# chanchanchan97/ICAFusion

Hardware: AMD Instinct MI355X
Metric: RGB/IR image-pairs/sec (two-stream forward + NMS) (higher is better)
Workload: dtype bf16

## Files before the change

### icafusion_amd/csrc/cstream.hip

```cpp
#include "conv_common.h"

namespace icaf {

constexpr int CS_C = 64, CS_TH = 8, CS_TW = 16, CS_HH = CS_TH + 2, CS_HWD = CS_TW + 2, CS_PITCH = 24;
constexpr int CS_NIDX = CS_HH * CS_PITCH;
constexpr int CS_PATCH = CS_NIDX * 128;
constexpr int CS_WBYTES = 9 * CS_C * 128;
constexpr int CS_W2BYTES = CS_C * 128;
constexpr int CS_SO = CS_C * 2 + 16;
constexpr int CS_STG = 128 * CS_SO;
constexpr int CS_LDS = CS_WBYTES + CS_W2BYTES + 2 * CS_PATCH + CS_STG;
static_assert(CS_LDS <= 160 * 1024, "LDS capacity");

struct CsGeom { int tiles_x, tiles_y, ntile; };

template <int DT, bool CHAIN>
__global__ __launch_bounds__(512) __attribute__((amdgpu_waves_per_eu(2, 2))) void cstream_kernel(const ConvP p, const CsGeom gm) {
    using E = Elem<DT>;
    static_assert(DT != ICAF_F32, "16-bit types");
    constexpr int RB = 128, NSTEP = 4, VEC = E::VEC;
    extern __shared__ __attribute__((aligned(1024))) unsigned char lds[];
    unsigned char* wbuf = lds;
    unsigned char* w2buf = lds + CS_WBYTES;
    unsigned char* patch0 = w2buf + CS_W2BYTES;
    unsigned char* stg = patch0 + 2 * CS_PATCH;

    const int tid = threadIdx.x, lane = tid & 63, l31 = lane & 31, hi = lane >> 5;
    const int wave = __builtin_amdgcn_readfirstlane(tid >> 6);
    const int g = blockIdx.z;
    const int wm = wave & 3, wn = wave >> 2;
    const int sy = wm >> 1, sx = wm & 1;

    const __amdgpu_buffer_rsrc_t xr = __builtin_amdgcn_make_buffer_rsrc(
        (void*)((const typename E::type*)p.x + g * p.x_gs), 0, p.x_bytes, 0x00020000);
    const __amdgpu_buffer_rsrc_t wr = __builtin_amdgcn_make_buffer_rsrc(
        (void*)((const typename E::type*)p.w + g * p.w_gs), 0, p.w_bytes, 0x00020000);
    constexpr unsigned OOB = 0x80000000u;

    {
        const int rsub = lane >> 3;
        for (int t = wave; t < 72; t += 8) {
            const int c = t >> 3, j = t & 7;
            const int sl = (lane & 7) ^ (((j & 1) << 2) | (rsub >> 1));
            const unsigned voff = ((unsigned)(j * 8 + rsub) * (unsigned)p.Kp + (unsigned)(c * 64 + sl * VEC)) * E::BYTES;
            __builtin_amdgcn_raw_ptr_buffer_load_lds(wr, (lds_ptr_t)(wbuf + (c * 64 + j * 8) * RB), 16, voff, 0, 0, 0);
        }
        if constexpr (CHAIN) {
            const __amdgpu_buffer_rsrc_t w2r = __builtin_amdgcn_make_buffer_rsrc(
                (void*)((const typename E::type*)p.w2 + g * p.w2_gs), 0, p.w2_bytes, 0x00020000);
            const int j = wave;
            const int sl = (lane & 7) ^ (((j & 1) << 2) | (rsub >> 1));
            const unsigned voff = ((unsigned)(j * 8 + rsub) * (unsigned)p.Kp2 + (unsigned)(sl * VEC)) * E::BYTES;
            __builtin_amdgcn_raw_ptr_buffer_load_lds(w2r, (lds_ptr_t)(w2buf + (j * 8) * RB), 16, voff, 0, 0, 0);
        }
    }

    const int xcd = blockIdx.x & 7, lb = blockIdx.x >> 3, wgx = gridDim.x >> 3;
    const int per_xcd = (gm.ntile + 7) >> 3, t_lo = xcd * per_xcd, t_hi = min(t_lo + per_xcd, gm.ntile);
    const int per_img = gm.tiles_x * gm.tiles_y;
    auto decode = [&](int t, int& b, int& y0, int& x0) {
        b = t / per_img;
        const int r = t - b * per_img, ty = r / gm.tiles_x;
        y0 = ty * CS_TH;
        x0 = (r - ty * gm.tiles_x) * CS_TW;
    };
    auto issue_patch = [&](int t, int buf) {
        int b, y0, x0;
        decode(t, b, y0, x0);
        const unsigned img_off = (unsigned)b * (unsigned)(p.H * p.W) * (unsigned)p.ldx * (unsigned)E::BYTES;
        unsigned char* dst = patch0 + buf * CS_PATCH;
        for (int j = wave; j < CS_PATCH / 1024; j += 8) {
            const int L = (j << 6) + lane, idx = L >> 3;
            const int cs = (L & 7) ^ ((idx >> 1) & 7);
            const int hy = idx / CS_PITCH, hx = idx - hy * CS_PITCH;
            const int gy = y0 - 1 + hy, gx = x0 - 1 + hx;
            const bool ok = hx < CS_HWD && (unsigned)gy < (unsigned)p.H && (unsigned)gx < (unsigned)p.W;
            const unsigned voff = ok ? img_off + (unsigned)((gy * p.W + gx) * p.ldx) * E::BYTES + (unsigned)(cs << 4) : OOB;
            __builtin_amdgcn_raw_ptr_buffer_load_lds(xr, (lds_ptr_t)(dst + (j << 10)), 16, voff, 0, 0, 0);
        }
    };

    f32x4 bq[4], bq2[4];
    {
        const float* __restrict__ bias = p.bias ? p.bias + g * p.bias_gs : nullptr;
        const float* __restrict__ bias2 = (CHAIN && p.bias2) ? p.bias2 + g * p.bias2_gs : nullptr;
#pragma unroll
        for (int qd = 0; qd < 4; ++qd) {
            const int n = wn * 32 + 8 * qd + 4 * hi;
            const f32x4 t1 = *(const f32x4*)((bias && n < p.Cout) ? bias + n : (const float*)p.w);
            bq[qd] = (bias && n < p.Cout) ? t1 : f32x4{0.f, 0.f, 0.f, 0.f};
            const f32x4 t2 = *(const f32x4*)((bias2 && n < p.Cout2) ? bias2 + n : (const float*)p.w);
            bq2[qd] = (bias2 && n < p.Cout2) ? t2 : f32x4{0.f, 0.f, 0.f, 0.f};
        }
#pragma unroll
        for (int qd = 0; qd < 4; ++qd) asm volatile("" : "+v"(bq[qd]), "+v"(bq2[qd]));
    }
    const int fkey = (l31 >> 1) & 7;
    int foff[NSTEP];
#pragma unroll
    for (int s = 0; s < NSTEP; ++s) foff[s] = (wn * 32 + l31) * RB + (((2 * s + hi) ^ fkey) << 4);
    const int lpy = sy * 4 + (l31 >> 3), lpx = sx * 8 + (l31 & 7);
    const int lbase = lpy * CS_PITCH + lpx;
    const int srow = wm * 32 + l31;

    int t = t_lo + lb;
    if (t >= t_hi) { wait_vmcnt<0>(); return; }
    issue_patch(t, 0);

    typename E::type* __restrict__ yg = (typename E::type*)p.y + g * p.y_gs;
    const typename E::type* __restrict__ rg = p.res ? (const typename E::type*)p.res + g * p.res_gs : nullptr;
    typename E::type* __restrict__ y2g = CHAIN ? (typename E::type*)p.y2 + g * p.y2_gs : nullptr;
    const float alpha_acc = p.alpha_acc[g], alpha_res = p.alpha_res[g];

    auto row_to_m = [&](int r, int b, int y0, int x0) {
        const int st = r >> 5, q = r & 31;
        const int gy = y0 + (st >> 1) * 4 + (q >> 3), gx = x0 + (st & 1) * 8 + (q & 7);
        return (gy < p.Ho && gx < p.Wo) ? (b * p.Ho + gy) * p.Wo + gx : -1;
    };
    u32x4 rres[2] = {u32x4{0u, 0u, 0u, 0u}, u32x4{0u, 0u, 0u, 0u}};
    auto flush = [&](typename E::type* dst, int ldd, int cout, int b, int y0, int x0, bool rr) {
#pragma unroll
        for (int it = 0; it < 2; ++it) {
            const int idx = tid + it * 512, row = idx >> 3, cv = idx & 7;
            const int m = row_to_m(row, b, y0, x0), n = cv * VEC;
            if (m >= 0 && n < cout) {
                u32x4 sv = *(const u32x4*)(stg + row * CS_SO + cv * 16);
                if (rr) {
                    float v[VEC], r[VEC];
                    unpack16<DT>(sv, v);
                    unpack16<DT>(rres[it], r);
#pragma unroll
                    for (int j = 0; j < VEC; ++j) v[j] = __builtin_fmaf(alpha_res, r[j], v[j]);
                    sv = pack16<DT>(v);
                }
                *(u32x4*)(dst + (long long)m * ldd + n) = sv;
            }
        }
    };
    auto load_res = [&](int b, int y0, int x0) {
#pragma unroll
        for (int it = 0; it < 2; ++it) {
            const int idx = tid + it * 512, row = idx >> 3, cv = idx & 7;
            const int m = row_to_m(row, b, y0, x0);
            rres[it] = *(const u32x4*)(rg + (long long)(m < 0 ? 0 : m) * p.ldr + cv * VEC);
        }
    };
    auto stage = [&](const f32x16& acc, const f32x4 (&bv)[4], float scale) {
#pragma unroll
        for (int qd = 0; qd < 4; ++qd) {
            const int nl = wn * 32 + 8 * qd + 4 * hi;
            float v[4];
#pragma unroll
            for (int j = 0; j < 4; ++j) v[j] = acc[4 * qd + j] + bv[qd][j] + 0.0f;
            silu4_f(v, v);
#pragma unroll
            for (int j = 0; j < 4; ++j) v[j] *= scale;
            u32x2 pk;
            if constexpr (DT == ICAF_BF16) { pk[0] = pack2_bf16(v[0], v[1]); pk[1] = pack2_bf16(v[2], v[3]); }
            else { pk[0] = pack2_f16(v[0], v[1]); pk[1] = pack2_f16(v[2], v[3]); }
            *(u32x2*)(stg + srow * CS_SO + nl * E::BYTES) = pk;
        }
    };

    int cur = 0, pb = -1, py0 = 0, px0 = 0;
    while (true) {
        int b, y0, x0;
        decode(t, b, y0, x0);
        const int tn = t + wgx;
        wait_vmcnt<0>();
        asm volatile("s_waitcnt lgkmcnt(0)" ::: "memory");
        __builtin_amdgcn_s_barrier();
        if (pb >= 0) {
            if constexpr (CHAIN) flush(y2g, p.ldy2, p.Cout2, pb, py0, px0, false);
            else flush(yg, p.ldy, p.Cout, pb, py0, px0, rg != nullptr);
        }
        if (rg) load_res(b, y0, x0);
        if (tn < t_hi) issue_patch(tn, cur ^ 1);
        const unsigned char* patch = patch0 + cur * CS_PATCH;
        f32x16 acc;
#pragma unroll
        for (int r = 0; r < 16; ++r) acc[r] = 0.0f;
#pragma unroll
        for (int c = 0; c < 9; ++c) {
            const int ky = c / 3, kx = c - 3 * ky;
            const int idx = lbase + ky * CS_PITCH + kx;
            const unsigned char* pe = patch + (idx << 7);
            const int key = (idx >> 1) & 7;
#pragma unroll
            for (int s = 0; s < NSTEP; ++s) {
                const u32x4 fp = *(const u32x4*)(pe + (((2 * s + hi) ^ key) << 4));
                const u32x4 fw = *(const u32x4*)(wbuf + c * (CS_C * RB) + foff[s]);
                mma_step<DT>(acc, fw, fp);
            }
        }
        lds_barrier();
        stage(acc, bq, alpha_acc);
        pb = b; py0 = y0; px0 = x0;
        if constexpr (CHAIN) {
            lds_barrier();
            if (rg) { wait_vmcnt<0>(); }
#pragma unroll
            for (int it = 0; it < 2; ++it) {
                const int idx = tid + it * 512, row = idx >> 3, cv = idx & 7;
                const int m = row_to_m(row, b, y0, x0), n = cv * VEC;
                if (m >= 0 && n < p.Cout) {
                    u32x4 sv = *(const u32x4*)(stg + row * CS_SO + cv * 16);
                    if (rg) {
                        float v[VEC], r[VEC];
                        unpack16<DT>(sv, v);
                        unpack16<DT>(rres[it], r);
#pragma unroll
                        for (int j = 0; j < VEC; ++j) v[j] = __builtin_fmaf(alpha_res, r[j], v[j]);
                        sv = pack16<DT>(v);
                        *(u32x4*)(stg + row * CS_SO + cv * 16) = sv;
                    }
                    if (p.keep1) *(u32x4*)(yg + (long long)m * p.ldy + n) = sv;
                }
            }
            lds_barrier();
            f32x16 acc2;
#pragma unroll
            for (int r = 0; r < 16; ++r) acc2[r] = 0.0f;
#pragma unroll
            for (int s = 0; s < NSTEP; ++s) {
                const u32x4 fp2 = *(const u32x4*)(stg + srow * CS_SO + ((2 * s + hi) << 4));
                const u32x4 fw2 = *(const u32x4*)(w2buf + foff[s]);
                mma_step<DT>(acc2, fw2, fp2);
            }
            lds_barrier();
            stage(acc2, bq2, 1.0f);
        }
        if (tn >= t_hi) break;
        t = tn;
        cur ^= 1;
    }
    wait_vmcnt<0>();
    lds_barrier();
    if constexpr (CHAIN) flush(y2g, p.ldy2, p.Cout2, pb, py0, px0, false);
    else flush(yg, p.ldy, p.Cout, pb, py0, px0, rg != nullptr);
}

const char* cstream_tag(int) { return "8x16n64"; }

int cstream_check(const icaf_conv_args* a, const ConvP& p, int) {
    if (a->dtype == ICAF_F32 || a->out_dtype != a->dtype) return fail(ICAF_ERR_UNSUPPORTED, "cstream: 16-bit types, out dtype == dtype");
    if (a->kh != 3 || a->kw != 3 || a->sh != 1 || a->sw != 1 || a->ph != 1 || a->pw != 1) return fail(ICAF_ERR_UNSUPPORTED, "cstream: 3x3 / stride 1 / pad 1 layers");
    if (a->Cin != CS_C || a->Cout > CS_C || a->Cout % 8 || a->Kp != 9 * CS_C) return fail(ICAF_ERR_UNSUPPORTED, "cstream: built for 64 -> (<= 64) channels (Cin = %d, Cout = %d, Kp = %d)", a->Cin, a->Cout, a->Kp);
    if (a->act != ICAF_ACT_SILU || a->pre) return fail(ICAF_ERR_UNSUPPORTED, "cstream: SiLU layers without a pre-activation term");
    if (p.x_bytes == 0) return fail(ICAF_ERR_UNSUPPORTED, "cstream: operand exceeds the 2 GiB buffer-descriptor range");
    if (!p.vec_y || (a->res && !p.vec_r)) return fail(ICAF_ERR_UNSUPPORTED, "cstream: y / res must take 16-byte vectors");
    if (a->w2) {
        if (a->Cout2 > CS_C || a->Cout2 % 8 || a->Kp2 != CS_C || !p.vec_y2 || a->Cout != CS_C) return fail(ICAF_ERR_UNSUPPORTED, "cstream: chained 1x1 of 64 -> (<= 64) channels with Kp2 = 64");
        if (a->res && !a->chain_keep) return fail(ICAF_ERR_UNSUPPORTED, "cstream: a residual needs chain_keep");
        if (a->chain_keep && (a->alpha_acc[0] != 1.0f || a->alpha_acc[1] != 1.0f)) return fail(ICAF_ERR_UNSUPPORTED, "cstream: chain_keep with alpha_acc != 1");
    }
    return ICAF_OK;
}

template <int DT, bool CHAIN>
static int launch_cstream_cfg(const ConvP& p, int groups, hipStream_t s) {
    CsGeom gm;
    gm.tiles_x = (p.Wo + CS_TW - 1) / CS_TW;
    gm.tiles_y = (p.Ho + CS_TH - 1) / CS_TH;
    gm.ntile = p.B * gm.tiles_x * gm.tiles_y;
    int dev = 0, cus = 256;
    ICAF_HIP(hipGetDevice(&dev));
    ICAF_HIP(hipDeviceGetAttribute(&cus, hipDeviceAttributeMultiprocessorCount, dev));
    int grid = (cus / groups) & ~7;
    if (grid < 8) grid = 8;
    ICAF_LDS_OPTIN((cstream_kernel<DT, CHAIN>), CS_LDS);
    cstream_kernel<DT, CHAIN><<<dim3((unsigned)grid, 1, (unsigned)groups), dim3(512), CS_LDS, s>>>(p, gm);
    ICAF_LAUNCH_CHECK();
    return ICAF_OK;
}

int launch_cstream(const icaf_conv_args* a, const ConvP& p, int, hipStream_t s) {
    if (a->dtype == ICAF_BF16) return a->w2 ? launch_cstream_cfg<ICAF_BF16, true>(p, a->groups, s) : launch_cstream_cfg<ICAF_BF16, false>(p, a->groups, s);
    return a->w2 ? launch_cstream_cfg<ICAF_F16, true>(p, a->groups, s) : launch_cstream_cfg<ICAF_F16, false>(p, a->groups, s);
}

}
```

Before: 16840.

## Incremental tile walk, precomputed patch/flush offsets, software-pipelined LDS fragment loads

Replaces the per-tile divide-based tile decode with an incremental walker, and precomputes the per-lane patch DMA and flush/residual offsets so each tile only adds a base offset. Unrolls the tile loop over two compile-time buffer indices so LDS addresses fold into immediates. Double-buffers the weight and patch fragment reads in the 9-tap MMA loop, prefetching the next tap's operands behind the current MFMA with sched barriers. It also adds an optional clock-stamp probe build and a phase-timing script. The aim is to cut scalar/VALU address overhead and hide LDS read latency, at the cost of more live VGPRs under a 2-waves-per-EU limit.

```diff
diff --git a/icafusion_amd/csrc/cs_walk.h b/icafusion_amd/csrc/cs_walk.h
--- /dev/null
+++ b/icafusion_amd/csrc/cs_walk.h
@@ -0,0 +1,94 @@
+#pragma once
+
+#if defined(__HIPCC__) || defined(__CUDACC__)
+#define ICAF_CS_HD __host__ __device__ __forceinline__
+#else
+#define ICAF_CS_HD inline
+#endif
+
+namespace icaf {
+
+constexpr int CSW_TH = 8, CSW_TW = 16, CSW_HH = CSW_TH + 2, CSW_HWD = CSW_TW + 2, CSW_PITCH = 24;
+constexpr int CSW_NDMA = CSW_HH * CSW_PITCH * 128 / 1024;
+constexpr int CSW_NEVER = 0x40000000;
+constexpr unsigned CSW_OOB = 0x80000000u;
+
+struct CsWalk {
+    int t, t_hi, stride;
+    int img, ty, tx;
+    int s_img, s_ty, s_tx;
+    int tiles_x, tiles_y;
+};
+
+ICAF_CS_HD bool cs_walk_start(CsWalk& w, int ntile, int tiles_x, int tiles_y, int xcd, int lb, int wgx) {
+    const int per_xcd = (ntile + 7) >> 3, t_lo = xcd * per_xcd;
+    w.t_hi = t_lo + per_xcd < ntile ? t_lo + per_xcd : ntile;
+    w.t = t_lo + lb;
+    w.stride = wgx;
+    w.tiles_x = tiles_x;
+    w.tiles_y = tiles_y;
+    if (w.t >= w.t_hi) return false;
+    const int per_img = tiles_x * tiles_y;
+    w.img = w.t / per_img;
+    int r = w.t - w.img * per_img;
+    w.ty = r / tiles_x;
+    w.tx = r - w.ty * tiles_x;
+    w.s_img = wgx / per_img;
+    r = wgx - w.s_img * per_img;
+    w.s_ty = r / tiles_x;
+    w.s_tx = r - w.s_ty * tiles_x;
+    return true;
+}
+
+ICAF_CS_HD bool cs_walk_has_next(const CsWalk& w) { return w.t + w.stride < w.t_hi; }
+
+ICAF_CS_HD void cs_walk_next(CsWalk& w) {
+    w.t += w.stride;
+    w.tx += w.s_tx;
+    if (w.tx >= w.tiles_x) { w.tx -= w.tiles_x; ++w.ty; }
+    w.ty += w.s_ty;
+    if (w.ty >= w.tiles_y) { w.ty -= w.tiles_y; ++w.img; }
+    w.img += w.s_img;
+}
+
+struct CsPatchLane {
+    int hy1, hx1;
+    unsigned rel;
+};
+
+ICAF_CS_HD CsPatchLane cs_patch_lane(int j, int lane, int W, int pix_bytes) {
+    const int L = (j << 6) + lane, idx = L >> 3;
+    const int cs = (L & 7) ^ ((idx >> 1) & 7);
+    const int hy = idx / CSW_PITCH, hx = idx - hy * CSW_PITCH;
+    CsPatchLane pl;
+    pl.hy1 = hy - 1;
+    pl.hx1 = hx < CSW_HWD ? hx - 1 : CSW_NEVER;
+    pl.rel = hx < CSW_HWD ? (unsigned)((pl.hy1 * W + pl.hx1) * pix_bytes) + (unsigned)(cs << 4) : 0u;
+    return pl;
+}
+
+ICAF_CS_HD unsigned cs_tile_off(int img, int y0, int x0, int H, int W, int pix_bytes) {
+    return ((unsigned)img * (unsigned)(H * W) + (unsigned)(y0 * W + x0)) * (unsigned)pix_bytes;
+}
+
+ICAF_CS_HD unsigned cs_patch_voff(const CsPatchLane& pl, unsigned tile_off, int y0, int x0, int H, int W) {
+    const bool ok = (unsigned)(y0 + pl.hy1) < (unsigned)H && (unsigned)(x0 + pl.hx1) < (unsigned)W;
+    return ok ? tile_off + pl.rel : CSW_OOB;
+}
+
+struct CsFlushLane { int dy, dx, cv; };
+
+ICAF_CS_HD CsFlushLane cs_flush_lane(int tid, int it) {
+    const int idx = tid + it * 512, row = idx >> 3, st = row >> 5, q = row & 31;
+    return CsFlushLane{(st >> 1) * 4 + (q >> 3), (st & 1) * 8 + (q & 7), idx & 7};
+}
+
+ICAF_CS_HD int cs_frag_direct(int lbase, int ky, int kx, int s, int hi) {
+    const int idx = lbase + ky * CSW_PITCH + kx;
+    return (idx << 7) + (((2 * s + hi) ^ ((idx >> 1) & 7)) << 4);
+}
+ICAF_CS_HD int cs_frag_base(int lbase, int kx, int s, int hi) { return cs_frag_direct(lbase, 0, kx, s, hi); }
+constexpr int cs_frag_sel(int ky, int s) { return (ky & 1) ? (s ^ 2) : s; }
+constexpr int cs_frag_imm(int ky) { return ky * CSW_PITCH * 128; }
+
+}
diff --git a/icafusion_amd/csrc/cstream.hip b/icafusion_amd/csrc/cstream.hip
--- a/icafusion_amd/csrc/cstream.hip
+++ b/icafusion_amd/csrc/cstream.hip
@@ -1,8 +1,13 @@
 #include "conv_common.h"
+#include "cs_walk.h"
+#include <type_traits>
+#ifdef ICAF_CS_CLK
+#include <cstdlib>
+#endif
 
 namespace icaf {
 
-constexpr int CS_C = 64, CS_TH = 8, CS_TW = 16, CS_HH = CS_TH + 2, CS_HWD = CS_TW + 2, CS_PITCH = 24;
+constexpr int CS_C = 64, CS_TH = CSW_TH, CS_TW = CSW_TW, CS_HH = CSW_HH, CS_HWD = CSW_HWD, CS_PITCH = CSW_PITCH;
 constexpr int CS_NIDX = CS_HH * CS_PITCH;
 constexpr int CS_PATCH = CS_NIDX * 128;
 constexpr int CS_WBYTES = 9 * CS_C * 128;
@@ -11,8 +16,21 @@
 constexpr int CS_STG = 128 * CS_SO;
 constexpr int CS_LDS = CS_WBYTES + CS_W2BYTES + 2 * CS_PATCH + CS_STG;
 static_assert(CS_LDS <= 160 * 1024, "LDS capacity");
-
-struct CsGeom { int tiles_x, tiles_y, ntile; };
+static_assert(CS_PATCH == CSW_NDMA * 1024, "patch DMA instructions");
+
+struct CsGeom {
+    int tiles_x, tiles_y, ntile;
+#ifdef ICAF_CS_CLK
+    unsigned long long* clk;
+#endif
+};
+
+#ifdef ICAF_CS_CLK
+constexpr int CS_CLK_TILES = 16, CS_CLK_N = 8;
+#define CS_STAMP(i) do { if (blockIdx.x == 0 && blockIdx.z == 0 && lane == 0 && clk_tile < CS_CLK_TILES) gm.clk[(wave * CS_CLK_TILES + clk_tile) * CS_CLK_N + (i)] = __builtin_amdgcn_s_memtime(); } while (0)
+#else
+#define CS_STAMP(i) do { } while (0)
+#endif
 
 template <int DT, bool CHAIN>
 __global__ __launch_bounds__(512) __attribute__((amdgpu_waves_per_eu(2, 2))) void cstream_kernel(const ConvP p, const CsGeom gm) {
@@ -24,6 +42,7 @@
     unsigned char* w2buf = lds + CS_WBYTES;
     unsigned char* patch0 = w2buf + CS_W2BYTES;
     unsigned char* stg = patch0 + 2 * CS_PATCH;
+    constexpr int PATCH0 = CS_WBYTES + CS_W2BYTES;
 
     const int tid = threadIdx.x, lane = tid & 63, l31 = lane & 31, hi = lane >> 5;
     const int wave = __builtin_amdgcn_readfirstlane(tid >> 6);
@@ -35,7 +54,6 @@
         (void*)((const typename E::type*)p.x + g * p.x_gs), 0, p.x_bytes, 0x00020000);
     const __amdgpu_buffer_rsrc_t wr = __builtin_amdgcn_make_buffer_rsrc(
         (void*)((const typename E::type*)p.w + g * p.w_gs), 0, p.w_bytes, 0x00020000);
-    constexpr unsigned OOB = 0x80000000u;
 
     {
         const int rsub = lane >> 3;
@@ -55,29 +73,20 @@
         }
     }
 
-    const int xcd = blockIdx.x & 7, lb = blockIdx.x >> 3, wgx = gridDim.x >> 3;
-    const int per_xcd = (gm.ntile + 7) >> 3, t_lo = xcd * per_xcd, t_hi = min(t_lo + per_xcd, gm.ntile);
-    const int per_img = gm.tiles_x * gm.tiles_y;
-    auto decode = [&](int t, int& b, int& y0, int& x0) {
-        b = t / per_img;
-        const int r = t - b * per_img, ty = r / gm.tiles_x;
-        y0 = ty * CS_TH;
-        x0 = (r - ty * gm.tiles_x) * CS_TW;
-    };
-    auto issue_patch = [&](int t, int buf) {
-        int b, y0, x0;
-        decode(t, b, y0, x0);
-        const unsigned img_off = (unsigned)b * (unsigned)(p.H * p.W) * (unsigned)p.ldx * (unsigned)E::BYTES;
-        unsigned char* dst = patch0 + buf * CS_PATCH;
-        for (int j = wave; j < CS_PATCH / 1024; j += 8) {
-            const int L = (j << 6) + lane, idx = L >> 3;
-            const int cs = (L & 7) ^ ((idx >> 1) & 7);
-            const int hy = idx / CS_PITCH, hx = idx - hy * CS_PITCH;
-            const int gy = y0 - 1 + hy, gx = x0 - 1 + hx;
-            const bool ok = hx < CS_HWD && (unsigned)gy < (unsigned)p.H && (unsigned)gx < (unsigned)p.W;
-            const unsigned voff = ok ? img_off + (unsigned)((gy * p.W + gx) * p.ldx) * E::BYTES + (unsigned)(cs << 4) : OOB;
-            __builtin_amdgcn_raw_ptr_buffer_load_lds(xr, (lds_ptr_t)(dst + (j << 10)), 16, voff, 0, 0, 0);
-        }
+    CsWalk wk;
+    const bool any = cs_walk_start(wk, gm.ntile, gm.tiles_x, gm.tiles_y, blockIdx.x & 7, blockIdx.x >> 3, gridDim.x >> 3);
+
+    const int pixb = p.ldx * E::BYTES;
+    CsPatchLane pl[4];
+#pragma unroll
+    for (int k = 0; k < 4; ++k) pl[k] = cs_patch_lane(wave + 8 * k, lane, p.W, pixb);
+    auto issue_patch = [&](int b, int y0, int x0, int buf) {
+        const unsigned tile_off = cs_tile_off(b, y0, x0, p.H, p.W, pixb);
+        unsigned char* dst = patch0 + buf * CS_PATCH + (wave << 10);
+#pragma unroll
+        for (int k = 0; k < 4; ++k)
+            if (k < 3 || wave < CSW_NDMA - 24)
+                __builtin_amdgcn_raw_ptr_buffer_load_lds(xr, (lds_ptr_t)(dst + (k << 13)), 16, cs_patch_voff(pl[k], tile_off, y0, x0, p.H, p.W), 0, 0, 0);
     };
 
     f32x4 bq[4], bq2[4];
@@ -102,29 +111,51 @@
     const int lpy = sy * 4 + (l31 >> 3), lpx = sx * 8 + (l31 & 7);
     const int lbase = lpy * CS_PITCH + lpx;
     const int srow = wm * 32 + l31;
-
-    int t = t_lo + lb;
-    if (t >= t_hi) { wait_vmcnt<0>(); return; }
-    issue_patch(t, 0);
+    int wfo[2][NSTEP], pfo[3][NSTEP];
+#pragma unroll
+    for (int s = 0; s < NSTEP; ++s) {
+        wfo[0][s] = foff[s];
+        wfo[1][s] = foff[s] + 8 * (CS_C * RB);
+        asm volatile("" : "+v"(wfo[0][s]), "+v"(wfo[1][s]));
+#pragma unroll
+        for (int kx = 0; kx < 3; ++kx) {
+            pfo[kx][s] = PATCH0 + cs_frag_base(lbase, kx, s, hi);
+            asm volatile("" : "+v"(pfo[kx][s]));
+        }
+    }
+
+    if (!any) { wait_vmcnt<0>(); return; }
+    issue_patch(wk.img, wk.ty * CS_TH, wk.tx * CS_TW, 0);
 
     typename E::type* __restrict__ yg = (typename E::type*)p.y + g * p.y_gs;
     const typename E::type* __restrict__ rg = p.res ? (const typename E::type*)p.res + g * p.res_gs : nullptr;
     typename E::type* __restrict__ y2g = CHAIN ? (typename E::type*)p.y2 + g * p.y2_gs : nullptr;
     const float alpha_acc = p.alpha_acc[g], alpha_res = p.alpha_res[g];
 
-    auto row_to_m = [&](int r, int b, int y0, int x0) {
-        const int st = r >> 5, q = r & 31;
-        const int gy = y0 + (st >> 1) * 4 + (q >> 3), gx = x0 + (st & 1) * 8 + (q & 7);
-        return (gy < p.Ho && gx < p.Wo) ? (b * p.Ho + gy) * p.Wo + gx : -1;
-    };
+    typename E::type* __restrict__ const og = CHAIN ? y2g : yg;
+    const int ldo = CHAIN ? p.ldy2 : p.ldy;
+    const int fcv = tid & 7, fn = fcv * VEC;
+    const bool n_out = fn < (CHAIN ? p.Cout2 : p.Cout), n_y = fn < p.Cout;
+    int fdy[2], fdx[2], fo_out[2], fo_y[2], fo_r[2];
+#pragma unroll
+    for (int it = 0; it < 2; ++it) {
+        const CsFlushLane fl = cs_flush_lane(tid, it);
+        fdy[it] = fl.dy;
+        fdx[it] = fl.dx;
+        const int rel = fl.dy * p.Wo + fl.dx;
+        fo_out[it] = rel * ldo + fn;
+        fo_y[it] = rel * p.ldy + fn;
+        fo_r[it] = rel * p.ldr + fn;
+    }
+    struct TileOut { int m0, ny, nx; };
+    auto tile_out = [&](int b, int y0, int x0) { return TileOut{(b * p.Ho + y0) * p.Wo + x0, p.Ho - y0, p.Wo - x0}; };
     u32x4 rres[2] = {u32x4{0u, 0u, 0u, 0u}, u32x4{0u, 0u, 0u, 0u}};
-    auto flush = [&](typename E::type* dst, int ldd, int cout, int b, int y0, int x0, bool rr) {
+    auto flush = [&](const TileOut& to, bool rr) {
+        const long long base = (long long)to.m0 * ldo;
 #pragma unroll
         for (int it = 0; it < 2; ++it) {
-            const int idx = tid + it * 512, row = idx >> 3, cv = idx & 7;
-            const int m = row_to_m(row, b, y0, x0), n = cv * VEC;
-            if (m >= 0 && n < cout) {
-                u32x4 sv = *(const u32x4*)(stg + row * CS_SO + cv * 16);
+            if (n_out && fdy[it] < to.ny && fdx[it] < to.nx) {
+                u32x4 sv = *(const u32x4*)(stg + ((tid >> 3) + it * 64) * CS_SO + fcv * 16);
                 if (rr) {
                     float v[VEC], r[VEC];
                     unpack16<DT>(sv, v);
@@ -133,16 +164,16 @@
                     for (int j = 0; j < VEC; ++j) v[j] = __builtin_fmaf(alpha_res, r[j], v[j]);
                     sv = pack16<DT>(v);
                 }
-                *(u32x4*)(dst + (long long)m * ldd + n) = sv;
+                *(u32x4*)(og + (base + fo_out[it])) = sv;
             }
         }
     };
-    auto load_res = [&](int b, int y0, int x0) {
+    auto load_res = [&](const TileOut& to) {
+        const long long base = (long long)to.m0 * p.ldr;
 #pragma unroll
         for (int it = 0; it < 2; ++it) {
-            const int idx = tid + it * 512, row = idx >> 3, cv = idx & 7;
-            const int m = row_to_m(row, b, y0, x0);
-            rres[it] = *(const u32x4*)(rg + (long long)(m < 0 ? 0 : m) * p.ldr + cv * VEC);
+            const bool in = n_y && fdy[it] < to.ny && fdx[it] < to.nx;
+            rres[it] = *(const u32x4*)(rg + (in ? base + fo_r[it] : 0ll));
         }
     };
     auto stage = [&](const f32x16& acc, const f32x4 (&bv)[4], float scale) {
@@ -162,49 +193,66 @@
         }
     };
 
-    int cur = 0, pb = -1, py0 = 0, px0 = 0;
-    while (true) {
-        int b, y0, x0;
-        decode(t, b, y0, x0);
-        const int tn = t + wgx;
+    bool staged = false;
+    TileOut prev{0, 0, 0};
+#ifdef ICAF_CS_CLK
+    int clk_tile = -1;
+#endif
+    auto tile = [&](auto BUFC) -> bool {
+        constexpr int BUF = decltype(BUFC)::value;
+        const TileOut cur = tile_out(wk.img, wk.ty * CS_TH, wk.tx * CS_TW);
+        const bool more = cs_walk_has_next(wk);
+        cs_walk_next(wk);
+#ifdef ICAF_CS_CLK
+        ++clk_tile;
+#endif
+        CS_STAMP(0);
         wait_vmcnt<0>();
         asm volatile("s_waitcnt lgkmcnt(0)" ::: "memory");
         __builtin_amdgcn_s_barrier();
-        if (pb >= 0) {
-            if constexpr (CHAIN) flush(y2g, p.ldy2, p.Cout2, pb, py0, px0, false);
-            else flush(yg, p.ldy, p.Cout, pb, py0, px0, rg != nullptr);
-        }
-        if (rg) load_res(b, y0, x0);
-        if (tn < t_hi) issue_patch(tn, cur ^ 1);
-        const unsigned char* patch = patch0 + cur * CS_PATCH;
+        CS_STAMP(1);
+        if (staged) flush(prev, !CHAIN && rg != nullptr);
+        CS_STAMP(2);
+        if (rg) load_res(cur);
+        CS_STAMP(3);
+        if (more) issue_patch(wk.img, wk.ty * CS_TH, wk.tx * CS_TW, BUF ^ 1);
+        CS_STAMP(4);
         f32x16 acc;
 #pragma unroll
         for (int r = 0; r < 16; ++r) acc[r] = 0.0f;
+        u32x4 fwv[2][NSTEP], fpv[2][NSTEP];
+        auto rd = [&](int c, int s) {
+            const int ky = c / 3, kx = c - 3 * ky;
+            fwv[c & 1][s] = *(const u32x4*)(lds + (wfo[c >> 3][s] + (c & 7) * (CS_C * RB)));
+            fpv[c & 1][s] = *(const u32x4*)(lds + (pfo[kx][cs_frag_sel(ky, s)] + (cs_frag_imm(ky) + BUF * CS_PATCH)));
+        };
+#pragma unroll
+        for (int s = 0; s < NSTEP; ++s) rd(0, s);
+        __builtin_amdgcn_sched_barrier(0);
 #pragma unroll
         for (int c = 0; c < 9; ++c) {
-            const int ky = c / 3, kx = c - 3 * ky;
-            const int idx = lbase + ky * CS_PITCH + kx;
-            const unsigned char* pe = patch + (idx << 7);
-            const int key = (idx >> 1) & 7;
 #pragma unroll
             for (int s = 0; s < NSTEP; ++s) {
-                const u32x4 fp = *(const u32x4*)(pe + (((2 * s + hi) ^ key) << 4));
-                const u32x4 fw = *(const u32x4*)(wbuf + c * (CS_C * RB) + foff[s]);
-                mma_step<DT>(acc, fw, fp);
+                mma_step<DT>(acc, fwv[c & 1][s], fpv[c & 1][s]);
+                if (c < 8) rd(c + 1, s);
+                __builtin_amdgcn_sched_barrier(0);
             }
         }
+        CS_STAMP(5);
         lds_barrier();
         stage(acc, bq, alpha_acc);
-        pb = b; py0 = y0; px0 = x0;
+        prev = cur;
+        staged = true;
+        CS_STAMP(6);
         if constexpr (CHAIN) {
             lds_barrier();
             if (rg) { wait_vmcnt<0>(); }
+            const long long ybase = (long long)cur.m0 * p.ldy;
 #pragma unroll
             for (int it = 0; it < 2; ++it) {
-                const int idx = tid + it * 512, row = idx >> 3, cv = idx & 7;
-                const int m = row_to_m(row, b, y0, x0), n = cv * VEC;
-                if (m >= 0 && n < p.Cout) {
-                    u32x4 sv = *(const u32x4*)(stg + row * CS_SO + cv * 16);
+                if (n_y && fdy[it] < cur.ny && fdx[it] < cur.nx) {
+                    unsigned char* sp = stg + ((tid >> 3) + it * 64) * CS_SO + fcv * 16;
+                    u32x4 sv = *(const u32x4*)sp;
                     if (rg) {
                         float v[VEC], r[VEC];
                         unpack16<DT>(sv, v);
@@ -212,9 +260,9 @@
 #pragma unroll
                         for (int j = 0; j < VEC; ++j) v[j] = __builtin_fmaf(alpha_res, r[j], v[j]);
                         sv = pack16<DT>(v);
-                        *(u32x4*)(stg + row * CS_SO + cv * 16) = sv;
+                        *(u32x4*)sp = sv;
                     }
-                    if (p.keep1) *(u32x4*)(yg + (long long)m * p.ldy + n) = sv;
+                    if (p.keep1) *(u32x4*)(yg + (ybase + fo_y[it])) = sv;
                 }
             }
             lds_barrier();
@@ -230,14 +278,13 @@
             lds_barrier();
             stage(acc2, bq2, 1.0f);
         }
-        if (tn >= t_hi) break;
-        t = tn;
-        cur ^= 1;
-    }
+        CS_STAMP(7);
+        return more;
+    };
+    while (tile(std::integral_constant<int, 0>{}) && tile(std::integral_constant<int, 1>{})) { }
     wait_vmcnt<0>();
     lds_barrier();
-    if constexpr (CHAIN) flush(y2g, p.ldy2, p.Cout2, pb, py0, px0, false);
-    else flush(yg, p.ldy, p.Cout, pb, py0, px0, rg != nullptr);
+    flush(prev, !CHAIN && rg != nullptr);
 }
 
 const char* cstream_tag(int) { return "8x16n64"; }
@@ -263,6 +310,10 @@
     gm.tiles_x = (p.Wo + CS_TW - 1) / CS_TW;
     gm.tiles_y = (p.Ho + CS_TH - 1) / CS_TH;
     gm.ntile = p.B * gm.tiles_x * gm.tiles_y;
+#ifdef ICAF_CS_CLK
+    gm.clk = (unsigned long long*)strtoull(getenv("ICAF_S2_CLK_PTR") ? getenv("ICAF_S2_CLK_PTR") : "0", nullptr, 0);
+    if (!gm.clk) return fail(ICAF_ERR_ARG, "cstream probe build: ICAF_S2_CLK_PTR is not set");
+#endif
     int dev = 0, cus = 256;
     ICAF_HIP(hipGetDevice(&dev));
     ICAF_HIP(hipDeviceGetAttribute(&cus, hipDeviceAttributeMultiprocessorCount, dev));
diff --git a/lab/probes/cstream_phases.py b/lab/probes/cstream_phases.py
--- /dev/null
+++ b/lab/probes/cstream_phases.py
@@ -0,0 +1,38 @@
+import math, os, sys
+R = os.path.dirname(os.path.dirname(os.path.dirname(os.path.abspath(__file__)))); sys.path.insert(0, R)
+import torch
+DEV = "cuda:0"
+NT, NS = 16, 8
+clk = torch.zeros((8, NT, NS), dtype=torch.int64, device=DEV)
+os.environ["ICAF_S2_CLK_PTR"] = hex(clk.data_ptr())
+from icafusion_amd import ops
+dt, B, H, W, C = torch.bfloat16, 32, 80, 80, 64
+mk = lambda shape, s=1.0: torch.randn(shape, device=DEV) * s
+names = ["wait + barrier", "flush t-1", "residual", "patch issue", "K loop", "barrier + stage", "chain", "-> next tile"]
+for what, G, use_res, chain in (("3x3 + shortcut g=2", 2, True, False), ("3x3 + shortcut + chained 1x1 g=2", 2, True, True), ("3x3 g=1", 1, False, False)):
+    lead = (G, B, H, W) if G == 2 else (B, H, W)
+    x = mk(lead + (C,)).to(dt)
+    wp, kp, bp = ops.pack_streams([(mk((C, C, 3, 3), 1.0 / math.sqrt(9 * C)), mk((C,), 0.2)) for _ in range(G)], dt)
+    y = mk(lead + (C,)).to(dt)
+    ch = None
+    if chain:
+        w2p, kp2, b2p = ops.pack_streams([(mk((C, C, 1, 1), 1.0 / math.sqrt(C)), mk((C,), 0.2)) for _ in range(G)], dt)
+        ch = dict(w=w2p, kp=kp2, bias=b2p, y=torch.empty(lead + (C,), dtype=dt, device=DEV), cout=C, keep=True)
+    l = ops.conv2d(x, wp, kp, bp, y, 3, 3, 1, 1, 1, 1, C, C, ops.ACT_SILU, res=y if use_res else None, alpha_res=1.0 if use_res else 0.0, tile=71, chain=ch)
+    sp = ops.current_stream_ptr()
+    for _ in range(3): l(sp)
+    torch.cuda.synchronize()
+    e0, e1 = ops.Event(), ops.Event(); e0.record(sp)
+    for _ in range(20): l(sp)
+    e1.record(sp); torch.cuda.synchronize()
+    print(f"{what}: {e0.elapsed_ms(e1) / 20 * 1e3:7.1f} us  ({ops.conv_kernel_name(l)})")
+    c = clk.cpu().numpy()
+    if not c.any():
+        continue
+    for w in range(8):
+        d = c[w, 1:6, 1:] - c[w, 1:6, :-1]
+        nxt = c[w, 2:7, 0] - c[w, 1:6, 7]
+        seg = list(d.mean(0)) + [nxt.mean()]
+        tile = (c[w, 2:7, 0] - c[w, 1:6, 0]).mean()
+        print(f"  wave {w}: tile {tile:7.0f} cycles | " + " | ".join(f"{n} {v:5.0f}" for n, v in zip(names, seg)))
+    clk.zero_()
```

Measured after the change: 16950, median of 6. Within noise of the previous version (+0.7%).
